# FocoosAI/focoos

Measured on AMD Instinct MI355X. Metric: images/sec @ 640^2 (infer bs=32), higher is better.
Workload: dtype bf16; 1 GPU; fai-detr-l-obj365 inference, bf16 MFMA, bs=32/GPU, 640x640, random-init weights (seed 0), uint8 HWC images resident in HBM, device post-process + D2H of packed detections included; global_batch=32, parallelism=replicas x1 (no data-path collective), steps_are=hipGraph replays, batches_in_flight=3, concurrent_batch_parts=1

## Files before the change

focoos_amd/_lib.py:

```python
from __future__ import annotations

import ctypes as C
import os
from typing import Optional

from .build import LIB_PATH, LIB_PATH_FP16

FX_ACT = {None: 0, "none": 0, "relu": 1, "silu": 2, "gelu": 3}


class FocoosAmdError(RuntimeError):
    pass


class FxConvDesc(C.Structure):
    _fields_ = [
        ("x", C.c_void_p), ("w", C.c_void_p), ("bias", C.c_void_p), ("residual", C.c_void_p), ("y", C.c_void_p),
        ("B", C.c_int32), ("H", C.c_int32), ("W", C.c_int32), ("C", C.c_int32), ("ldx", C.c_int32),
        ("Ho", C.c_int32), ("Wo", C.c_int32), ("N", C.c_int32), ("ldy", C.c_int32), ("ldr", C.c_int32),
        ("KH", C.c_int32), ("KW", C.c_int32), ("stride", C.c_int32), ("pad", C.c_int32),
        ("pool2", C.c_int32), ("act", C.c_int32), ("out_f32", C.c_int32), ("residual_after_act", C.c_int32),
        ("y_batch_stride", C.c_int64), ("w_frag", C.c_void_p), ("mask", C.c_void_p), ("ldm", C.c_int32), ("reserved0", C.c_int32),
    ]

# ... 22 lines not shown
        ("w_fwd_frag", C.c_void_p), ("w_dgrad_frag", C.c_void_p), ("bias_out", C.c_void_p),
        ("N", C.c_int32), ("C", C.c_int32), ("KH", C.c_int32), ("KW", C.c_int32), ("ld_fwd", C.c_int32), ("ld_dgrad", C.c_int32),
        ("first_block", C.c_int32), ("n_offset", C.c_int32), ("n_total", C.c_int32), ("reserved", C.c_int32),
    ]


class FxPublishEntry(C.Structure):
    _fields_ = [
        ("w", C.c_void_p), ("bn_weight", C.c_void_p), ("bn_bias", C.c_void_p), ("bn_mean", C.c_void_p), ("bn_var", C.c_void_p),
        ("bias", C.c_void_p), ("w_rows", C.c_void_p), ("w_frag", C.c_void_p), ("bias_out", C.c_void_p), ("eps", C.c_double),
        ("N", C.c_int32), ("C", C.c_int32), ("KH", C.c_int32), ("KW", C.c_int32), ("Np", C.c_int32), ("first_block", C.c_int32),
    ]


class FxPwChainDesc(C.Structure):
    _fields_ = [
        ("x1", C.c_void_p), ("x2", C.c_void_p), ("residual", C.c_void_p), ("w1", C.c_void_p), ("bias1", C.c_void_p), ("y1", C.c_void_p),
        ("w2", C.c_void_p), ("bias2", C.c_void_p), ("y2", C.c_void_p),
        ("M", C.c_int32), ("K1a", C.c_int32), ("K1b", C.c_int32), ("N1", C.c_int32), ("N2", C.c_int32),
        ("ldx1", C.c_int32), ("ldx2", C.c_int32), ("ldr", C.c_int32), ("ldy1", C.c_int32), ("ldy2", C.c_int32),
        ("act1", C.c_int32), ("act2", C.c_int32),
        ("pool", C.c_void_p), ("ldp", C.c_int32), ("img_h", C.c_int32), ("img_w", C.c_int32), ("reserved0", C.c_int32),
    ]


class FxRcStage(C.Structure):
    _fields_ = [
        ("type", C.c_int32), ("K", C.c_int32), ("N", C.c_int32), ("act", C.c_int32),
        ("src", C.c_int32), ("dst", C.c_int32), ("aux", C.c_int32),
        ("ld", C.c_int32), ("ld2", C.c_int32), ("flags", C.c_int32),
        ("w", C.c_void_p), ("bias", C.c_void_p), ("gamma", C.c_void_p), ("beta", C.c_void_p), ("g0", C.c_void_p), ("g1", C.c_void_p),
    ]


class FxFrameDesc(C.Structure):
    _fields_ = [
        ("plane", C.c_void_p * 3), ("pitch", C.c_int32 * 3), ("height", C.c_int32), ("width", C.c_int32), ("format", C.c_int32),
        ("matrix", C.c_int32), ("reserved", C.c_int32 * 3),
    ]


_vp, _i, _f = C.c_void_p, C.c_int, C.c_float

SIGNATURES = {
    "fx_abi_version": [],
    "fx_build_flags": [],
    "fx_device_info": [_i, C.POINTER(C.c_int), C.c_char_p, _i],
    "fx_conv2d_nhwc_bf16": [C.POINTER(FxConvDesc), _vp],
    "fx_conv2d_variant": [_vp, C.c_char_p, _i],
    "fx_pw_chain_supported": [_i, _i, _i, _i],
    "fx_pw_chain_pool_supported": [_i, _i, _i, _i],
    "fx_conv3x3_flat_supported": [_i, _i, _i],
    "fx_pw_chain_bf16": [C.POINTER(FxPwChainDesc), _vp],
    "fx_stem_conv3x3s2": [_vp, _i, _vp, _vp, _vp, _vp, _vp, _i, _i, _i, _i, _vp],
    "fx_stem16_conv3x3s2": [_vp, _i, _vp, _vp, _vp, _vp, _vp, _i, _i, _i, _vp],
    "fx_conv3x3_c16_nhwc_bf16": [_vp, _i, _vp, _vp, _i, _vp, _i, _i, _i, _i, _i, _i, _i, _vp],
    "fx_semseg_eval_accumulate": [_vp, _vp, _i, _i, _i, _i, _i, _i, _i, _vp, C.c_int64, _vp, _vp, _i, _i, _vp, _vp, _vp, _vp, _vp],
    "fx_detr_eval_boxes_f32": [_vp, _vp, _vp, _i, _i, _i, _i, _vp, _vp, _vp, _vp, _vp],
    "fx_coco_match_workspace_bytes": [_i],
    "fx_coco_match_bbox": [_vp, _vp, _vp, _vp, _i, _i, _i, _vp, _vp, _vp, _vp, _vp, _vp, C.c_int64, _i, _vp, _vp, _vp, _vp, _vp, _vp, C.c_size_t,
                           _vp],
    "fx_mf_eval_masks_workspace_bytes": [_i, _i, _i],
    "fx_mf_eval_masks": [_vp, _vp, _vp, _i, _i, _i, _i, _i, _i, _i, _i, _vp, _vp, _vp, _vp, C.c_int64, _f, _vp, _vp, _vp, _vp, _vp, _vp, _vp, _vp,
                         _vp, _vp, C.c_size_t, _vp],
    "fx_coco_mask_inter": [_vp, _vp, _vp, C.c_int64, _vp, _vp, _vp, _i, _i, _i, _vp, _vp, _vp, _vp, _vp, C.c_int64, _vp, _vp, _vp, C.c_int64, _vp,
                           _vp, _vp],
    "fx_coco_match_segm": [_vp, _vp, _vp, _vp, _i, _i, _i, _i, _vp, _vp, _vp, _vp, _vp, _vp, _vp, C.c_int64, _i, _vp, _vp, _vp, _vp, _vp, _vp,
                           C.c_size_t, _vp],
    "fx_augment_images_u8": [_vp, _vp, _vp, _vp, _vp, C.c_int64, _vp, _vp, _i, _vp, _i, _i, _i, _vp, _vp],
    "fx_augment_labels": [_vp, _vp, _vp, _vp, _vp, _vp, C.c_int64, _vp, _vp, _vp, _i, _i, _vp, _i, _i, _i, _i, _vp, _vp],
    "fx_resize_bilinear_u8": [_vp, _i, _i, _vp, _i, _i, _vp],
    "fx_tile_gather_u8_f32": [_vp, _i, _i, _vp, _vp, _i, _vp, _i, _i, _vp],
    "fx_frames_ingest": [_vp, _vp, _i, _vp, _i, _i, _i, _vp],
    "fx_merge_detections_workspace_bytes": [_i, _i],
    "fx_merge_detections_nms": [_vp, _vp, _vp, _vp, _vp, _i, _i, _i, _i, _f, _i, _i, _vp, _vp, _vp, _vp, _vp, _vp, C.c_size_t, _vp],
    "fx_frames_tile_gather_f32": [_vp, _vp, _i, _vp, _vp, _i, _vp, _i, _i, _vp],
    "fx_roi_select": [_vp, _vp, _vp, _vp, _i, _i, _vp, _vp, _i, _vp, _vp, _vp, _vp, _vp, _vp, _i, _i, _i, _i, _f, _i, _vp, _vp, _vp, _vp, _vp],
    "fx_frames_roi_gather_f32": [_vp, _vp, _i, _vp, _i, _vp, _i, _i, _vp],
    "fx_roi_attributes": [_vp, _i, _vp, _vp, _i, _vp, _i, _i, _vp, _vp, _i, _vp, _vp, _vp, _vp, _vp, _i, _vp, _vp, _vp, _vp],
    "fx_merge_detections_batched_workspace_bytes": [_i, _i, _i],
    "fx_merge_detections_nms_batched": [_vp, _vp, _vp, _vp, _vp, _i, _i, _i, _i, _i, _f, _i, _i, _vp, _vp, _vp, _vp, _vp, _vp, C.c_size_t, _vp],
    "fx_annotate_labels_from_detections": [_vp, _vp, _vp, _vp, _i, _i, _vp, _vp, _i, _i, _i, _i, _i, _i, _vp, _vp],
    "fx_annotate_u8": [_vp, _vp, _i, _i, _i, _i, _i, _vp, _vp, _vp, _vp, _vp, _i, C.c_int64, _vp, _vp, _i, _i, _i, _i, _vp],
    "fx_track_update": [_vp, _vp, _vp, _vp, _i, _i, _vp, _vp, _vp, _vp, _vp, _vp, _vp, _vp, _i, _f, _f, _f, _f, _f, _i, _i, _f, _vp, _vp],
    "fx_track_reset": [_vp, _vp, _vp, _vp, _vp, _vp, _vp, _vp, _i, _i, _i, _vp],
    "fx_zone_update": [_vp, _vp, _vp, _i, _i, _vp, _vp, _i, _vp, _vp, _vp, _vp, _vp, _vp, _i, _i, _vp, _vp, _vp, _vp, _vp, _vp, _vp, _vp, _vp],
    "fx_zone_reset": [_vp, _vp, _vp, _vp, _vp, _i, _i, _i, _i, _vp],
    "fx_annotate_labels_tracked": [_vp, _vp, _vp, _vp, _vp, _i, _i, _vp, _vp, _i, _i, _i, _i, _i, _i, _vp, _vp],
    "fx_annotate_zone_records": [_vp, _vp, _vp, _vp, _vp, _vp, _i, _i, _vp, _vp, _vp, _vp, _vp, _i, _i, _i, _i, _i, _i, _vp, _vp],
    "fx_annotate_overlay_u8": [_vp, _vp, _i, _i, _i, _i, _i, _vp, _vp, _vp, _vp, _vp, _vp, _i, _i, _vp, _vp, _vp, _vp, _vp, _vp, _i, _i, _i, _i,
                               _vp],
    "fx_trace_update": [_vp, _vp, _vp, _i, _i, _vp, _vp, _i, _i, _vp, _vp, _vp, _vp, _vp, _vp],
    "fx_trace_reset": [_vp, _vp, _vp, _vp, _i, _i, _i, _vp],
    "fx_dwell_update": [_vp, _vp, _vp, _i, _i, _vp, _i, _vp, _vp, _vp, _vp, _vp, _vp, _i, _vp, _vp, _vp, _vp, _vp, _vp, _vp, _vp, _vp],
    "fx_dwell_reset": [_vp, _vp, _vp, _vp, _vp, _vp, _vp, _vp, _i, _i, _i, _i, _vp],
    "fx_heat_tiles": [_i, _i, _i],
    "fx_heat_update": [_vp, _vp, _vp, _vp, _i, _i, _i, _i, _i, _i, _i, _i, _i, _vp, _vp, _vp, _vp, _vp],
    "fx_annotate_heat_u8": [_vp, _vp, _i, _i, _i, _i, _i, _vp, _vp, _i, _i, _vp, _vp],
    "fx_redact_regions": [_vp, _vp, _vp, _i, _i, _vp, _i, _vp, _vp, _vp, _vp, _i, _i, _i, _i, _vp, _vp, _vp, _vp],
    "fx_redact_u8": [_vp, _vp, _i, _i, _i, _i, _vp, _vp, _vp, _i, _vp, _i, C.c_int64, _i, _i, _i, _i, _i, _i, _vp],
    "fx_mask_rle_workspace_bytes": [_i, _i, _i, _i],
    "fx_mask_rle_encode": [_vp, _vp, _vp, _i, _i, _i, _i, _i, _vp, _vp, _vp, _vp, C.c_size_t, _vp],
    "fx_mask_polygon_workspace_bytes": [_i, _i, _i, _i, _i],
    "fx_mask_polygon_encode": [_vp, _vp, _vp, _i, _i, _i, _i, _i, _i, _vp, _vp, _vp, _vp, C.c_size_t, _vp],
    "fx_maxpool3x3s2_nhwc_bf16": [_vp, _i, _vp, _i, _i, _i, _i, _i, _vp],
    "fx_stem_conv12_u8_bf16": [_vp, _vp, _vp, _vp, _vp, _vp, _vp, _vp, _i, _i, _i, _i, _vp],
# ... 228 lines not shown
```

focoos_amd/csrc/conv_pw_chain.hip:

```cpp
#include "pw_common.h"

struct PwChainArgs {
  const bf16_t* x1;
  const bf16_t* x2;
  const bf16_t* res;
  const bf16_t* w1p;
  const bf16_t* w2p;
  const float* b1;
  const float* b2;
  bf16_t* y1;
  bf16_t* y2;
  int ldx1, ldx2, ldr, ldy1, ldy2;
  int M, N1, act1, act2;
  unsigned x1_bytes, x2_bytes, r_bytes;
  bf16_t* pool;
  int ldp, H, W;
};

template <int RL, typename F>
__device__ __forceinline__ void pw_dma_rows_map(__amdgpu_buffer_rsrc_t r, unsigned char* tile, int nrows, int ld, int col0, int wave, int lane, F&& pix) {
  const int ninstr = nrows * RL / 64;
  for (int i = wave; i < ninstr; i += 4) {
    const int q = i * 64 + lane;
    const int row = q / RL, pc = q % RL;
    const int lc = pw_swz<RL>(row, pc);
    const int m = pix(row);
    const unsigned off = (m >= 0) ? (unsigned)(m * ld + col0 + lc * 8) * 2u : FX_OOB;
    pw_dma16(r, tile + i * 1024, off);
  }
}

template <int K1A, int K1B, int N2, int BM, bool QUAD = false>
__global__ __launch_bounds__(256, ((N2 <= 64 && K1B == 0) ? 4 : ((N2 <= 128 && (K1B == 0 || N2 <= 64)) ? 3 : 2))) void pw_chain_kernel(const PwChainArgs p) {
  constexpr int K1 = K1A + K1B, KS1 = K1 / 16, KS1A = K1A / 16;
  constexpr int RLA = K1A / 8, RLB = (K1B > 0 ? K1B : 64) / 8;
  constexpr int TM = BM / 32;
  constexpr int XA_BYTES = BM * K1A * 2, XB_BYTES = BM * K1B * 2;
  constexpr int PF1 = KS1 < 4 ? KS1 : 4;
  constexpr bool HAS2 = N2 > 0;
  constexpr int WN2 = !HAS2 ? 1 : (N2 >= 128 ? 4 : 2), WM2 = 4 / WN2;
  constexpr int TN2 = !HAS2 ? 1 : N2 / (32 * WN2), TM2 = BM / (32 * WM2);
  constexpr int RL2 = (HAS2 ? N2 : 64) / 8;
  constexpr int PF2 = 4;
  static_assert(BM == 64, "64-pixel tiles");
  static_assert(K1A % 64 == 0 && K1B % 64 == 0 && PF1 == 4, "K segments in multiples of 64 (= whole blocks of 4 k-steps)");
  static_assert(!HAS2 || (N2 % 64 == 0 && N2 <= 256), "N2");
  extern __shared__ __attribute__((aligned(16))) unsigned char smem[];
  unsigned char* XA = smem;
  unsigned char* XB = smem + XA_BYTES;
  unsigned char* T = smem + XA_BYTES + XB_BYTES;

  const int tid = threadIdx.x, lane = tid & 63;
  const int wave = __builtin_amdgcn_readfirstlane(tid >> 6);
  const int l32 = lane & 31, half = lane >> 5;
  const int m0 = blockIdx.x * BM;
  const int NG = p.N1 >> 8;
  const int KS2 = p.N1 >> 4;

  __shared__ int s_pix[QUAD ? BM : 1];
  if constexpr (QUAD) {
    if (tid < BM) {
      const int W2 = p.W >> 1, QI = (p.H >> 1) * W2;
      const int q = blockIdx.x * (BM / 4) + (tid >> 2), sub = tid & 3;
      int m = -1;
      if (q * 4 < p.M) {
        const int b = q / QI, rem = q - b * QI;
        const int y2 = rem / W2, x2 = rem - y2 * W2;
        m = (b * p.H + 2 * y2 + (sub >> 1)) * p.W + 2 * x2 + (sub & 1);
      }
      s_pix[tid] = m;
    }
    __syncthreads();
  }
  auto pix = [&](int row) -> int {
    if constexpr (!QUAD) {
      const int m = m0 + row;
      return m < p.M ? m : -1;
    } else {
      return s_pix[row];
    }
  };
  const __amdgpu_buffer_rsrc_t x1r = __builtin_amdgcn_make_buffer_rsrc((void*)p.x1, 0, p.x1_bytes, 0x00020000);
  pw_dma_rows_map<RLA>(x1r, XA, BM, p.ldx1, 0, wave, lane, pix);
  if constexpr (K1B > 0) {
    const __amdgpu_buffer_rsrc_t x2r = __builtin_amdgcn_make_buffer_rsrc((void*)p.x2, 0, p.x2_bytes, 0x00020000);
    pw_dma_rows_map<RLB>(x2r, XB, BM, p.ldx2, 0, wave, lane, pix);
  }
  const __amdgpu_buffer_rsrc_t rr = __builtin_amdgcn_make_buffer_rsrc((void*)(p.res ? p.res : p.x1), 0, p.res ? p.r_bytes : 0u, 0x00020000);

  const int wn2 = wave % WN2, wm2 = wave / WN2;
  f32x16 acc2[TN2][TM2];
#pragma unroll
  for (int a = 0; a < TN2; ++a)
#pragma unroll
    for (int b = 0; b < TM2; ++b)
#pragma unroll
      for (int r = 0; r < 16; ++r) acc2[a][b][r] = 0.0f;

  for (int g = 0; g < NG; ++g) {
    int l32g = l32, halfg = half, tidg = tid;
    asm volatile("" : "+v"(l32g), "+v"(halfg), "+v"(tidg));
    if (p.res) pw_dma_rows_map<32>(rr, T, BM, p.ldr, g * 256, wave, lane, pix);
    bf16x8 a2[PF2][TN2];
    const bf16_t* w2 = p.w2p + (size_t)((wn2 * TN2) * KS2 + g * 16) * 512 + lane * 8;
    if constexpr (HAS2) {
#pragma unroll
      for (int i = 0; i < PF2; ++i)
#pragma unroll
        for (int a = 0; a < TN2; ++a) a2[i][a] = pw_ldg_frag(w2 + (size_t)(a * KS2 + i) * 512);
    }
#pragma unroll
    for (int a = 0; a < 2; ++a) {
      const bf16_t* w1 = p.w1p + (size_t)((g * 8 + wave * 2 + a) * KS1) * 512 + lane * 8;
      bf16x8 a1[PF1];
#pragma unroll
      for (int i = 0; i < PF1; ++i) a1[i] = pw_ldg_frag(w1 + i * 512);
      f32x16 acc[TM];
#pragma unroll
      for (int gq = 0; gq < 4; ++gq) {
        const float4 bb = *reinterpret_cast<const float4*>(p.b1 + g * 256 + wave * 64 + a * 32 + 8 * gq + 4 * halfg);
#pragma unroll
        for (int b = 0; b < TM; ++b) {
          acc[b][4 * gq] = bb.x; acc[b][4 * gq + 1] = bb.y; acc[b][4 * gq + 2] = bb.z; acc[b][4 * gq + 3] = bb.w;
        }
      }
      if (a == 0) {
        asm volatile("s_waitcnt vmcnt(0)" ::: "memory");
        __syncthreads();
      }
#define FX_PW_STEPS(XT_, KROW_, RL_, KL0_)                                                                                  \
  _Pragma("unroll") for (int i = 0; i < PF1; ++i) {                                                                         \
    bf16x8 xb[TM];                                                                                                          \
    _Pragma("unroll") for (int b = 0; b < TM; ++b) {                                                                        \
      const int row = b * 32 + l32k;                                                                                         \
      xb[b] = *reinterpret_cast<const bf16x8*>((XT_) + row * ((KROW_)*2) + (pw_swz<RL_>(row, ((KL0_) + i) * 2 + halfg) << 4)); \
    }                                                                                                                       \
    _Pragma("unroll") for (int b = 0; b < TM; ++b) acc[b] = FX_MFMA_32x32x16(a1[i], xb[b], acc[b]); \
    const int kn = ks0 + i + PF1;                                                                                           \
    a1[i] = pw_ldg_frag(w1 + (kn < KS1 ? kn : KS1 - 1) * 512);  \
  }
#pragma unroll 1
      for (int ks0 = 0; ks0 < KS1; ks0 += PF1) {
        int l32k = l32g;
        asm volatile("" : "+v"(l32k));
        if (K1B == 0 || ks0 < KS1A) {
          FX_PW_STEPS(XA, K1A, RLA, ks0)
        } else {
          FX_PW_STEPS(XB, (K1B > 0 ? K1B : 64), RLB, ks0 - KS1A)
        }
      }
#undef FX_PW_STEPS
#pragma unroll
      for (int b = 0; b < TM; ++b)
#pragma unroll
        for (int gq = 0; gq < 4; ++gq) {
          const int row = b * 32 + l32g;
          const int chunk = wave * 8 + a * 4 + gq;
          unsigned char* tp = T + row * 512 + ((chunk ^ (row & 15)) << 4) + halfg * 8;
          float v0 = acc[b][4 * gq], v1 = acc[b][4 * gq + 1], v2 = acc[b][4 * gq + 2], v3 = acc[b][4 * gq + 3];
          if (p.res) {
            const uint2 r2 = *reinterpret_cast<const uint2*>(tp);
            v0 += bf16lo_to_f32(r2.x);
            v1 += bf16hi_to_f32(r2.x);
            v2 += bf16lo_to_f32(r2.y);
            v3 += bf16hi_to_f32(r2.y);
          }
          if (p.act1 == FX_ACT_RELU) {
            v0 = fmaxf(v0, 0.0f); v1 = fmaxf(v1, 0.0f); v2 = fmaxf(v2, 0.0f); v3 = fmaxf(v3, 0.0f);
          }
          uint2 o;
          o.x = pack_bf16x2(v0, v1);
          o.y = pack_bf16x2(v2, v3);
          *reinterpret_cast<uint2*>(tp) = o;
        }
    }
    __syncthreads();
#pragma unroll
    for (int i = 0; i < BM * 32 / 256; ++i) {
      const int q = tidg + i * 256;
      const int row = q >> 5, lc = q & 31;
      const uint4 v = *reinterpret_cast<const uint4*>(T + row * 512 + ((lc ^ (row & 15)) << 4));
      const int m = pix(row);
      if (m >= 0 && p.y1) *reinterpret_cast<uint4*>(p.y1 + (size_t)m * p.ldy1 + g * 256 + lc * 8) = v;
    }
    if constexpr (QUAD) {
#pragma unroll
      for (int i = 0; i < (BM / 4) * 32 / 256; ++i) {
        const int idx = tidg + i * 256;
        const int j = idx >> 5, lc = idx & 31;
        float s8[8] = {0, 0, 0, 0, 0, 0, 0, 0};
#pragma unroll
        for (int r = 0; r < 4; ++r) {
          const int row = 4 * j + r;
          float f[8];
          unpack_bf16x8(*reinterpret_cast<const uint4*>(T + row * 512 + ((lc ^ (row & 15)) << 4)), f);
#pragma unroll
          for (int e = 0; e < 8; ++e) s8[e] += f[e];
        }
#pragma unroll
        for (int e = 0; e < 8; ++e) s8[e] *= 0.25f;
        const int q = blockIdx.x * (BM / 4) + j;
        if (q * 4 < p.M) *reinterpret_cast<uint4*>(p.pool + (size_t)q * p.ldp + g * 256 + lc * 8) = pack_bf16x8(s8);
      }
    }
    if constexpr (HAS2) {
#pragma unroll
      for (int ks = 0; ks < 16; ++ks) {
        bf16x8 tb[TM2];
#pragma unroll
        for (int b = 0; b < TM2; ++b) {
          const int row = (wm2 * TM2 + b) * 32 + l32g;
          tb[b] = *reinterpret_cast<const bf16x8*>(T + row * 512 + (((ks * 2 + halfg) ^ (row & 15)) << 4));
        }
#pragma unroll
        for (int a = 0; a < TN2; ++a)
#pragma unroll
          for (int b = 0; b < TM2; ++b) acc2[a][b] = FX_MFMA_32x32x16(a2[ks % PF2][a], tb[b], acc2[a][b]);
        if (ks + PF2 < 16) {
#pragma unroll
          for (int a = 0; a < TN2; ++a) a2[ks % PF2][a] = pw_ldg_frag(w2 + (size_t)(a * KS2 + ks + PF2) * 512);
        }
      }
    }
    __syncthreads();
  }

  if constexpr (HAS2) {
#pragma unroll
    for (int a = 0; a < TN2; ++a)
#pragma unroll
      for (int gq = 0; gq < 4; ++gq) {
        const int n = (wn2 * TN2 + a) * 32 + 8 * gq + 4 * half;
        const float4 bb = *reinterpret_cast<const float4*>(p.b2 + n);
#pragma unroll
        for (int b = 0; b < TM2; ++b) {
          const int row = (wm2 * TM2 + b) * 32 + l32;
          float v0 = acc2[a][b][4 * gq] + bb.x, v1 = acc2[a][b][4 * gq + 1] + bb.y;
          float v2 = acc2[a][b][4 * gq + 2] + bb.z, v3 = acc2[a][b][4 * gq + 3] + bb.w;
          if (p.act2 == FX_ACT_RELU) {
            v0 = fmaxf(v0, 0.0f); v1 = fmaxf(v1, 0.0f); v2 = fmaxf(v2, 0.0f); v3 = fmaxf(v3, 0.0f);
          }
          uint2 o;
          o.x = pack_bf16x2(v0, v1);
          o.y = pack_bf16x2(v2, v3);
          *reinterpret_cast<uint2*>(T + row * (N2 * 2) + (pw_swz<RL2>(row, n >> 3) << 4) + half * 8) = o;
        }
      }
    __syncthreads();
#pragma unroll
    for (int i = 0; i < BM * RL2 / 256; ++i) {
      const int q = tid + i * 256;
      const int row = q / RL2, lc = q % RL2;
      const uint4 v = *reinterpret_cast<const uint4*>(T + row * (N2 * 2) + (pw_swz<RL2>(row, lc) << 4));
      const int m = pix(row);
      if (m >= 0) *reinterpret_cast<uint4*>(p.y2 + (size_t)m * p.ldy2 + lc * 8) = v;
    }
  }
}

template <int K1A, int K1B, int N2, bool QUAD = false>
static int launch_pw_chain(const PwChainArgs& a, hipStream_t stream) {
  constexpr int BM = 64;
  constexpr int SMEM = BM * (K1A + K1B) * 2 + BM * 512;
  auto kern = pw_chain_kernel<K1A, K1B, N2, BM, QUAD>;
  static int attr_smem = 0;
  if (!fx_ensure_dyn_smem(reinterpret_cast<const void*>(kern), SMEM, attr_smem)) return FX_ERR_RUNTIME;
  hipLaunchKernelGGL(kern, dim3((a.M + BM - 1) / BM), dim3(256), SMEM, stream, a);
  return fx_launch_status();
}

#define FX_PW_INSTANCES(X)                                                                             \
  X(64, 0, 0) X(64, 0, 64) X(64, 0, 128) X(64, 64, 0) X(64, 64, 64) X(64, 64, 128)                     \
  X(128, 0, 0) X(128, 0, 128) X(128, 0, 256) X(128, 256, 0) X(128, 256, 128) X(128, 256, 256)          \
  X(256, 0, 0) X(256, 0, 256) X(256, 512, 0) X(256, 512, 256)

extern "C" int fx_pw_chain_supported(int K1a, int K1b, int N1, int N2) {
  if (N1 <= 0 || N1 % 256 != 0) return 0;
#define FX_PW_CASE(KA, KB, NN2) \
  if (K1a == KA && K1b == KB && N2 == NN2) return 1;
  FX_PW_INSTANCES(FX_PW_CASE)
#undef FX_PW_CASE
  return 0;
}

#define FX_PW_POOL_INSTANCES(X) X(64, 0, 128) X(128, 0, 256)

extern "C" int fx_pw_chain_pool_supported(int K1a, int K1b, int N1, int N2) {
  if (N1 <= 0 || N1 % 256 != 0) return 0;
#define FX_PW_CASE(KA, KB, NN2) \
  if (K1a == KA && K1b == KB && N2 == NN2) return 1;
  FX_PW_POOL_INSTANCES(FX_PW_CASE)
#undef FX_PW_CASE
  return 0;
}

extern "C" int fx_pw_chain_bf16(const fx_pw_chain_desc* d, fx_stream_t stream_) {
  FX_CHECK_ARG(d && d->x1 && d->w1 && d->bias1 && d->M > 0);
  FX_CHECK_ARG(d->y1 || (d->pool && d->N2 > 0));
  FX_CHECK_ARG(d->K1b == 0 || d->x2);
  FX_CHECK_ARG((d->act1 == FX_ACT_NONE || d->act1 == FX_ACT_RELU) && (d->act2 == FX_ACT_NONE || d->act2 == FX_ACT_RELU));
  FX_CHECK_ARG(d->N2 == 0 || (d->w2 && d->bias2 && d->y2));
  if (!fx_pw_chain_supported(d->K1a, d->K1b, d->N1, d->N2)) return FX_ERR_UNSUPPORTED;
  FX_CHECK_ARG(d->ldx1 >= d->K1a && d->ldx1 % 8 == 0 && (!d->y1 || (d->ldy1 >= d->N1 && d->ldy1 % 8 == 0)));
  FX_CHECK_ARG(d->K1b == 0 || (d->ldx2 >= d->K1b && d->ldx2 % 8 == 0));
  FX_CHECK_ARG(!d->residual || (d->ldr >= d->N1 && d->ldr % 8 == 0));
  FX_CHECK_ARG(d->N2 == 0 || (d->ldy2 >= d->N2 && d->ldy2 % 8 == 0));
  FX_CHECK_ARG(((uintptr_t)d->x1 % 16) == 0 && ((uintptr_t)d->x2 % 16) == 0 && ((uintptr_t)d->residual % 16) == 0);
  FX_CHECK_ARG(((uintptr_t)d->w1 % 16) == 0 && ((uintptr_t)d->w2 % 16) == 0 && ((uintptr_t)d->y1 % 16) == 0 && ((uintptr_t)d->y2 % 16) == 0);
  FX_CHECK_ARG(((uintptr_t)d->bias1 % 16) == 0 && ((uintptr_t)d->bias2 % 16) == 0);
  const int64_t x1_bytes = ((int64_t)d->M - 1) * d->ldx1 * 2 + (int64_t)d->K1a * 2;
  const int64_t x2_bytes = d->K1b ? ((int64_t)d->M - 1) * d->ldx2 * 2 + (int64_t)d->K1b * 2 : 0;
  const int64_t r_bytes = d->residual ? ((int64_t)d->M - 1) * d->ldr * 2 + (int64_t)d->N1 * 2 : 0;
  if (x1_bytes >= 0xFFFFFFF0ll || x2_bytes >= 0xFFFFFFF0ll || r_bytes >= 0xFFFFFFF0ll) return FX_ERR_UNSUPPORTED;
  PwChainArgs a;
  a.x1 = reinterpret_cast<const bf16_t*>(d->x1);
  a.x2 = reinterpret_cast<const bf16_t*>(d->x2);
  a.res = reinterpret_cast<const bf16_t*>(d->residual);
  a.w1p = reinterpret_cast<const bf16_t*>(d->w1);
  a.w2p = reinterpret_cast<const bf16_t*>(d->w2);
  a.b1 = d->bias1;
  a.b2 = d->bias2;
  a.y1 = reinterpret_cast<bf16_t*>(d->y1);
  a.y2 = reinterpret_cast<bf16_t*>(d->y2);
  a.ldx1 = d->ldx1; a.ldx2 = d->ldx2; a.ldr = d->ldr; a.ldy1 = d->ldy1; a.ldy2 = d->ldy2;
  a.M = d->M; a.N1 = d->N1; a.act1 = d->act1; a.act2 = d->act2;
  a.x1_bytes = (unsigned)x1_bytes; a.x2_bytes = (unsigned)x2_bytes; a.r_bytes = (unsigned)r_bytes;
  a.pool = reinterpret_cast<bf16_t*>(d->pool); a.ldp = d->ldp; a.H = d->img_h; a.W = d->img_w;
  hipStream_t stream = reinterpret_cast<hipStream_t>(stream_);
  if (d->pool) {
    FX_CHECK_ARG(d->img_h > 0 && d->img_w > 0 && d->img_h % 2 == 0 && d->img_w % 2 == 0 && d->M % (d->img_h * d->img_w) == 0);
    FX_CHECK_ARG(d->ldp >= d->N1 && d->ldp % 8 == 0 && ((uintptr_t)d->pool % 16) == 0);
    if (!fx_pw_chain_pool_supported(d->K1a, d->K1b, d->N1, d->N2)) return FX_ERR_UNSUPPORTED;
#define FX_PW_CASE(KA, KB, NN2) \
  if (d->K1a == KA && d->K1b == KB && d->N2 == NN2) return launch_pw_chain<KA, KB, NN2, true>(a, stream);
    FX_PW_POOL_INSTANCES(FX_PW_CASE)
#undef FX_PW_CASE
    return FX_ERR_UNSUPPORTED;
  }
#define FX_PW_CASE(KA, KB, NN2) \
  if (d->K1a == KA && d->K1b == KB && d->N2 == NN2) return launch_pw_chain<KA, KB, NN2>(a, stream);
  FX_PW_INSTANCES(FX_PW_CASE)
#undef FX_PW_CASE
  return FX_ERR_UNSUPPORTED;
}
```

focoos_amd/engine.py:

```python
from __future__ import annotations

import contextlib
import ctypes as C
import functools
import math
import os
import weakref
from typing import Dict, List, Optional, Sequence, Tuple

import torch

from . import _lib
from ._lib import FX_ACT, FxConvDesc, FxPwChainDesc, FxRcStage, check
from .engine_stdc import StdcEngineMixin, StdcPlanMixin
from .state_spec import RESNET_BLOCKS

BN_EPS = 1e-5
DEFAULT_STREAMS = 2
MIN_PART_BATCH = 4
DEFAULT_PIPELINE_DEPTH = 3


def resolve_parts(B: int, nsplit: Optional[int], two_queue_safe: bool) -> int:
    if nsplit is None:
# ... 694 lines not shown
        d.x, d.w, d.bias = x.ptr, pc.w.data_ptr(), pc.b.data_ptr()
        d.residual = residual.ptr if residual is not None else None
        d.y = out.ptr
        d.B, d.H, d.W, d.C, d.ldx = x.B, x.H, x.W, x.C, x.ld
        d.Ho, d.Wo, d.N, d.ldy = Ho, Wo, pc.N, out.ld
        d.ldr = residual.ld if residual is not None else 0
        d.KH, d.KW, d.stride, d.pad = pc.KH, pc.KW, stride, pad
        d.pool2, d.act, d.out_f32 = int(pool2), FX_ACT[act], int(out_f32)
        d.residual_after_act = int(res_after)
        d.y_batch_stride = y_batch_stride
        d.w_frag = pc.wf.data_ptr() if pc.wf is not None else None
        self.keep.append(d)
        M = x.B * Ho * Wo
        flops = 2.0 * M * pc.N * pc.KH * pc.KW * pc.C + extra_flops_per_pixel * M
        label = C.create_string_buffer(64)
        check(self.lib.fx_conv2d_variant(C.byref(d), label, 64), "fx_conv2d_variant")
        variant = label.value.decode()
        alg_bytes = 2.0 * x.B * x.H * x.W * pc.C + (4.0 if out_f32 else 2.0) * M * pc.N + (2.0 * M * pc.N if residual is not None else 0.0) \
            + 2.0 * pc.N * pc.KH * pc.KW * pc.C
        self.meta[len(self.ops)] = {"kind": "conv", "variant": variant, "flops": flops, "flops_executed": flops - extra_flops_per_pixel * M, "bytes": alg_bytes,
                                    "name": name or "slice", "M": M, "N": pc.N, "K": pc.KH * pc.KW * pc.C}
        self._op(self.lib.fx_conv2d_nhwc_bf16, C.byref(d))
        return out

    def pw_chain(self, x1: NT, x2: Optional[NT], residual: Optional[NT], cc: Tuple, ca: Optional[Tuple], name1: str, name2: Optional[str],
                 pool_name: Optional[str] = None, keep_y1: bool = True):
        w1, b1, k1a, k1b, n1 = cc
        assert x1.C == k1a and (x2 is None) == (k1b == 0) and (x2 is None or x2.C == k1b), (name1, x1.C, k1a, k1b)
        M = x1.rows
        assert keep_y1 or (pool_name is not None and ca is not None)
        y1 = self._new(name1, x1.B, x1.H, x1.W, n1) if keep_y1 else None
        d = FxPwChainDesc()
        d.x1, d.ldx1, d.K1a = x1.ptr, x1.ld, k1a
        d.x2, d.ldx2, d.K1b = (x2.ptr, x2.ld, k1b) if x2 is not None else (None, 0, 0)
        d.residual, d.ldr = (residual.ptr, residual.ld) if residual is not None else (None, 0)
        d.w1, d.bias1, d.N1, d.M = w1.data_ptr(), b1.data_ptr(), n1, M
        d.y1, d.ldy1 = (y1.ptr, y1.ld) if y1 is not None else (None, 0)
        d.act1 = d.act2 = FX_ACT["relu"]
        y2, n2 = None, 0
        if ca is not None:
            w2, b2, n2 = ca
            y2 = self._new(name2, x1.B, x1.H, x1.W, n2)
            d.w2, d.bias2, d.y2, d.ldy2 = w2.data_ptr(), b2.data_ptr(), y2.ptr, y2.ld
        d.N2 = n2
        pooled = None
        if pool_name is not None:
            pooled = self._new(pool_name, x1.B, x1.H // 2, x1.W // 2, n1)
            d.pool, d.ldp, d.img_h, d.img_w = pooled.ptr, pooled.ld, x1.H, x1.W
        self.keep.append(d)
        self.meta[len(self.ops)] = {"kind": "conv", "variant": f"pw_chain<{k1a},{k1b},{n2}>" + ("+pool" if pooled is not None else "") + ("-y1" if y1 is None else ""),
                                    "flops": 2.0 * M * n1 * (k1a + k1b + n2),
                                    "name": name1 + ("+" + name2.rsplit("res_layers.", 1)[-1] if name2 else ""), "M": M, "N": n1, "K": k1a + k1b,
                                    "bytes": 2.0 * M * (k1a + k1b + (n1 if residual is not None else 0) + (n1 if y1 is not None else 0) + n2
                                                        + (n1 / 4 if pooled is not None else 0))}
        self._op(self.lib.fx_pw_chain_bf16, C.byref(d))
        if pool_name is not None:
            return y1, y2, pooled
        return y1, y2

    def linear(self, x: NT, pc: PackedConv, **kw) -> NT:
        return self.conv(x.as_rows() if (x.H != 1 or x.W != 1) else x, pc, **kw)

    def layernorm(self, x: NT, name_ln: str, out_name: str, residual: Optional[NT] = None) -> NT:
        g, b = self.eng.ln[name_ln]
        cols = int(g.numel())
        out = self._new(out_name, x.rows, 1, 1, cols)
        self._op(self.lib.fx_layernorm_bf16, x.ptr, x.ld, residual.ptr if residual is not None else None,
                 residual.ld if residual is not None else 0, g.data_ptr(), b.data_ptr(), out.ptr, out.ld, x.rows, cols)
        return out

    def add_rows(self, x: NT, y: NT, y_rows: int, out_name: str) -> NT:
        out = self._new(out_name, x.rows, 1, 1, x.C)
        self._op(self.lib.fx_add_rows_bf16, x.ptr, x.ld, y.ptr, y.ld, y_rows, out.ptr, out.ld, x.rows, x.C)
        return out

    RC_S0, RC_S1, RC_S2, RC_S3, RC_BIG, RC_REF, RC_RED, RC_LDS = 0, 16384, 32768, 49152, 65536, 131072, 131584, 132608
    RC2_REF, RC2_RED, RC2_LDS = 65536, 66048, 67072

    def _rc_program(self, stages: List[FxRcStage], rows: int, label: str, flops: float, lds: Optional[int] = None):
        arr = (FxRcStage * len(stages))(*stages)
        host = torch.frombuffer(bytearray(bytes(arr)), dtype=torch.uint8)
        dev = host.to(self.dev)
        self.keep.append(dev)
        self.meta[len(self.ops)] = {"kind": "conv", "variant": "row_chain", "flops": flops, "name": label, "M": rows, "N": 0, "K": 0}
        self._op(self.lib.fx_row_chain, dev.data_ptr(), len(stages), rows, self.RC_LDS if lds is None else lds)

    def resize(self, x: NT, out: NT):
        self._op(self.lib.fx_resize_bilinear_nhwc_bf16, x.ptr, x.ld, out.ptr, out.ld, x.B, x.H, x.W, x.C, out.H, out.W)

    def mha(self, qkv: NT, B: int, L: int, out_name: str) -> NT:
        out = self._new(out_name, B * L, 1, 1, 256)
        q, k, v = qkv.slice(0, 256), qkv.slice(256, 256), qkv.slice(512, 256)
        self._op(self.lib.fx_mha_bf16, q.ptr, q.ld, k.ptr, k.ld, v.ptr, v.ld, out.ptr, out.ld, B, L, L, 8)
        return out

    def build_backbone(self) -> Dict[int, NT]:
        e, P, B, lib = self.eng, self.eng.P, self.B, self.lib
        H, W = self.H, self.W
        bb = "pixel_decoder.backbone"
        self.input = self._io("input", (B, H, W, 3), torch.float32 if self.f32_input else torch.uint8)
        self.sizes = self._io("sizes", (B, 2), torch.int32)
        blocks = RESNET_BLOCKS[e.depth]
        feats = {}
        use_chain = int(os.environ.get("FX_PW_CHAIN", "1")) != 0
        max_stage = int(os.environ.get("FX_PW_CHAIN_MAX_STAGE", "1"))
        pc2 = P[f"{bb}.conv1.conv1_2"]
        if os.environ.get("FX_STEM12_FUSE", "1") != "0" and not self.f32_input and pc2.wf is not None and pc2.N == 32:
# ... 517 lines not shown
```

include/focoos_amd.h:

```cpp
#ifndef FOCOOS_AMD_H
#define FOCOOS_AMD_H

#include <stddef.h>
#include <stdint.h>

#ifdef __cplusplus
extern "C" {
#endif

#define FX_ABI_VERSION 27

enum { FX_OK = 0, FX_ERR_INVALID_ARGUMENT = -1, FX_ERR_LAUNCH = -2, FX_ERR_UNSUPPORTED = -3, FX_ERR_RUNTIME = -4 };
enum { FX_ACT_NONE = 0, FX_ACT_RELU = 1, FX_ACT_SILU = 2, FX_ACT_GELU = 3 };
enum { FX_CLASS_LOSS_CE = 0, FX_CLASS_LOSS_FOCAL = 1, FX_CLASS_LOSS_BCE = 2, FX_CLASS_LOSS_BCE_FOCAL = 3 };

typedef void* fx_stream_t;

int fx_abi_version(void);
int fx_build_flags(void);
const char* fx_error_string(int code);
int fx_device_info(int device, int* cu_count, char* arch_name, int arch_name_len);

typedef struct fx_conv_desc {
  const void* x;
  const void* w;
  const float* bias;
  const void* residual;
  void* y;
  int32_t B, H, W, C, ldx;
  int32_t Ho, Wo, N, ldy, ldr;
  int32_t KH, KW, stride, pad;
  int32_t pool2;
  int32_t act;
  int32_t out_f32;
  int32_t residual_after_act;
  int64_t y_batch_stride;
  const void* w_frag;
  const void* mask;
  int32_t ldm, reserved0;
} fx_conv_desc;
int fx_conv2d_nhwc_bf16(const fx_conv_desc* d, fx_stream_t stream);
int fx_conv2d_variant(const fx_conv_desc* d, char* out, int cap);
int fx_conv3x3_flat_supported(int C, int N, int W);

typedef struct fx_pw_chain_desc {
  const void* x1;
  const void* x2;
  const void* residual;
  const void* w1;
  const float* bias1;
  void* y1;
  const void* w2;
  const float* bias2;
  void* y2;
  int32_t M, K1a, K1b, N1, N2;
  int32_t ldx1, ldx2, ldr, ldy1, ldy2;
  int32_t act1, act2;
  void* pool;
  int32_t ldp, img_h, img_w, reserved0;
} fx_pw_chain_desc;
int fx_pw_chain_supported(int K1a, int K1b, int N1, int N2);
int fx_pw_chain_pool_supported(int K1a, int K1b, int N1, int N2);
int fx_pw_chain_bf16(const fx_pw_chain_desc* d, fx_stream_t stream);

int fx_stem_conv3x3s2(const void* x, int in_f32, const float* w, const float* bias, const float* mean,
                      const float* inv_std, void* y, int B, int H, int W, int Cout, fx_stream_t stream);

int fx_stem_conv12_u8_bf16(const void* x_u8, const float* w1, const float* b1, const float* mean, const float* inv_std, const void* w2_frag,
                           const float* b2, void* y, int ldy, int B, int H, int W, fx_stream_t stream);

int fx_stem16_conv3x3s2(const void* x, int in_f32, const float* w, const float* bias, const float* mean, const float* inv_std, void* y, int B,
                        int H, int W, fx_stream_t stream);
int fx_conv3x3_c16_nhwc_bf16(const void* x, int ldx, const void* w_frag, const float* bias, int relu, void* y, int ldy, int B, int H, int W, int C,
                             int N, int stride, fx_stream_t stream);

int fx_semseg_eval_accumulate(const float* mask_probs, const float* probs, int B, int Q, int K, int h, int w, int Hin, int Win, const int32_t* sizes,
                              int64_t max_pixels, const void* gt, const int64_t* gt_off, int gt_int32, int ignore_label, int64_t* conf,
                              int32_t* status, int32_t* pred, float* score, fx_stream_t stream);

int fx_detr_eval_boxes_f32(const int32_t* idx, const float* boxes, const int32_t* sizes, int B, int Q, int K, int T,
                           int32_t* label, float* xyxy, int32_t* keep, float* xywh, fx_stream_t stream);

size_t fx_coco_match_workspace_bytes(int max_gt);
int fx_coco_match_bbox(const int32_t* label, const float* score, const int32_t* keep, const float* xywh, int B, int T, int K,
                       const double* gt_box, const int32_t* gt_cat, const int32_t* gt_flag, const double* gt_area, const int64_t* gt_off,
                       const int64_t* gt_off_host, int64_t n_gt, int max_gt, int32_t* rank, uint64_t* matched, uint64_t* ignored,
                       int64_t* npig, int32_t* status, void* ws, size_t ws_bytes, fx_stream_t stream);

size_t fx_mf_eval_masks_workspace_bytes(int B, int Q, int max_h);
int fx_mf_eval_masks(const float* mask_probs, const float* val, const int32_t* idx, int B, int Q, int K, int T, int h, int w, int Hin, int Win,
                     const int32_t* sizes, const int32_t* sizes_host, const int64_t* word_off, const int64_t* word_off_host, int64_t n_words,
                     float mask_threshold, void* words, int32_t* qlist, int32_t* nref, int32_t* count, int32_t* box, float* psum, int32_t* label,
                     int32_t* query, float* score, void* ws, size_t ws_bytes, fx_stream_t stream);
int fx_coco_mask_inter(const void* words, const int64_t* word_off, const int64_t* word_off_host, int64_t n_words, const int32_t* qlist,
                       const int32_t* nref, const int32_t* box, int B, int Q, int T, const int32_t* sizes, const int32_t* sizes_host,
                       const void* gt_words, const int64_t* gt_word_off, const int64_t* gt_word_off_host, int64_t n_gt_words,
                       const int32_t* gt_box, const int64_t* gt_off, const int64_t* gt_off_host, int64_t n_gt, int32_t* inter, int32_t* gcount,
                       fx_stream_t stream);
int fx_coco_match_segm(const int32_t* label, const float* score, const int32_t* query, const int32_t* dcount, int B, int T, int K, int Q,
                       const int32_t* inter, const int32_t* gcount, const int32_t* gt_cat, const int32_t* gt_flag, const double* gt_area,
                       const int64_t* gt_off, const int64_t* gt_off_host, int64_t n_gt, int max_gt, int32_t* rank, uint64_t* matched,
                       uint64_t* ignored, int64_t* npig, int32_t* status, void* ws, size_t ws_bytes, fx_stream_t stream);

typedef struct fx_aug_record {
  int32_t crop_w, crop_h, pad_x, pad_y, res_w, res_h, crop_x, crop_y, flags, reserved0;
  float brightness, contrast, saturation;
  int32_t reserved1[3];
} fx_aug_record;

int fx_augment_images_u8(const uint8_t* src, const int64_t* src_off, const int32_t* sizes, const fx_aug_record* recs, const int64_t* src_off_host,
                         int64_t src_bytes, const int32_t* sizes_host, const fx_aug_record* recs_host, int B, uint8_t* dst, int Ho, int Wo,
                         int pad_value, uint64_t* mean_ws, fx_stream_t stream);

int fx_augment_labels(const void* src, const int64_t* src_off, const int32_t* plane_rec, const int32_t* sizes, const fx_aug_record* recs,
                      const int64_t* src_off_host, int64_t src_count, const int32_t* plane_rec_host, const int32_t* sizes_host,
                      const fx_aug_record* recs_host, int P, int B, void* dst, int Ho, int Wo, int elem_int32, int pad_value, int32_t* flags,
// ... 501 lines not shown
```

Baseline: 5113 images/s.

## Add 128-pixel tile variant for pointwise chain kernel on large-M layers

Adds a BM=128 variant of the fused pointwise-chain kernel that processes N1 in 128-column groups instead of 256, with its own occupancy calculation and staging layout. A heuristic picks the bigger tile for specific shapes (K1a=64,N2=64 unpooled or K1a=128,N2=256 pooled) when M is at least 65536. The aim is to reuse each weight fragment load across twice as many pixels, cutting weight traffic per output. The cost is more LDS and register use per block, so fewer blocks can be resident on a CU, and the number of kernel template instances grows.

Result: slower. 5057 images/s (-1.1%).

```diff
diff --git a/focoos_amd/_lib.py b/focoos_amd/_lib.py
--- a/focoos_amd/_lib.py
+++ b/focoos_amd/_lib.py
@@ -98,6 +98,9 @@
     "fx_pw_chain_pool_supported": [_i, _i, _i, _i],
     "fx_conv3x3_flat_supported": [_i, _i, _i],
     "fx_pw_chain_bf16": [C.POINTER(FxPwChainDesc), _vp],
+    "fx_pw_chain_tile": [_i, _i, _i, _i, _i, _i],
+    "fx_pw_chain_bf16_tile": [C.POINTER(FxPwChainDesc), _i, _vp],
+    "fx_pw_chain_last_tile": [],
     "fx_stem_conv3x3s2": [_vp, _i, _vp, _vp, _vp, _vp, _vp, _i, _i, _i, _i, _vp],
     "fx_stem16_conv3x3s2": [_vp, _i, _vp, _vp, _vp, _vp, _vp, _i, _i, _i, _vp],
     "fx_conv3x3_c16_nhwc_bf16": [_vp, _i, _vp, _vp, _i, _vp, _i, _i, _i, _i, _i, _i, _i, _vp],
diff --git a/focoos_amd/csrc/conv_pw_chain.hip b/focoos_amd/csrc/conv_pw_chain.hip
--- a/focoos_amd/csrc/conv_pw_chain.hip
+++ b/focoos_amd/csrc/conv_pw_chain.hip
@@ -15,6 +15,7 @@
   unsigned x1_bytes, x2_bytes, r_bytes;
   bf16_t* pool;
   int ldp, H, W;
+  int wmask;
 };
 
 template <int RL, typename F>
@@ -30,8 +31,16 @@
   }
 }
 
-template <int K1A, int K1B, int N2, int BM, bool QUAD = false>
-__global__ __launch_bounds__(256, ((N2 <= 64 && K1B == 0) ? 4 : ((N2 <= 128 && (K1B == 0 || N2 <= 64)) ? 3 : 2))) void pw_chain_kernel(const PwChainArgs p) {
+template <int K1A, int K1B, int N2, int BM>
+constexpr int pw_chain_occupancy() {
+  if (BM == 64) return (N2 <= 64 && K1B == 0) ? 4 : ((N2 <= 128 && (K1B == 0 || N2 <= 64)) ? 3 : 2);
+  const int lds = (160 * 1024) / (BM * (K1A + K1B) * 2 + 32 * 1024);
+  const int regs = N2 <= 64 ? 3 : ((K1A == 64 && K1B > 0) ? 1 : 2);
+  return lds < regs ? lds : regs;
+}
+
+template <int K1A, int K1B, int N2, int BM, bool QUAD = false, int ABL = 0>
+__global__ __launch_bounds__(256, (pw_chain_occupancy<K1A, K1B, N2, BM>())) void pw_chain_kernel(const PwChainArgs p) {
   constexpr int K1 = K1A + K1B, KS1 = K1 / 16, KS1A = K1A / 16;
   constexpr int RLA = K1A / 8, RLB = (K1B > 0 ? K1B : 64) / 8;
   constexpr int TM = BM / 32;
@@ -41,20 +50,32 @@
   constexpr int WN2 = !HAS2 ? 1 : (N2 >= 128 ? 4 : 2), WM2 = 4 / WN2;
   constexpr int TN2 = !HAS2 ? 1 : N2 / (32 * WN2), TM2 = BM / (32 * WM2);
   constexpr int RL2 = (HAS2 ? N2 : 64) / 8;
-  constexpr int PF2 = 4;
-  static_assert(BM == 64, "64-pixel tiles");
+  constexpr int PF2 = (BM == 128 && N2 == 256 && K1B == 0) ? 2 : 4;
+  constexpr int GC = BM == 64 ? 256 : 128;
+  constexpr int RLT = GC / 8, TROW = GC * 2;
+  constexpr int RLT_LOG = BM == 64 ? 5 : 4, GC_LOG = RLT_LOG + 3;
+  constexpr int NPASS = GC / 128;
+  constexpr int KSG = GC / 16;
+  constexpr int T_BYTES = BM * TROW;
+  static_assert(BM == 64 || BM == 128, "64- or 128-pixel tiles");
   static_assert(K1A % 64 == 0 && K1B % 64 == 0 && PF1 == 4, "K segments in multiples of 64 (= whole blocks of 4 k-steps)");
   static_assert(!HAS2 || (N2 % 64 == 0 && N2 <= 256), "N2");
   extern __shared__ __attribute__((aligned(16))) unsigned char smem[];
   unsigned char* XA = smem;
   unsigned char* XB = smem + XA_BYTES;
   unsigned char* T = smem + XA_BYTES + XB_BYTES;
+  unsigned char* Y2T = (BM * N2 * 2 <= T_BYTES) ? T : smem;
+  static_assert(BM * N2 * 2 <= T_BYTES || BM * N2 * 2 <= XA_BYTES + XB_BYTES + T_BYTES, "y2 staging tile");
 
   const int tid = threadIdx.x, lane = tid & 63;
   const int wave = __builtin_amdgcn_readfirstlane(tid >> 6);
   const int l32 = lane & 31, half = lane >> 5;
   const int m0 = blockIdx.x * BM;
-  const int NG = p.N1 >> 8;
+  const int NG = p.N1 >> GC_LOG;
+  auto widx = [&](int i) -> int {
+    if constexpr (ABL != 0) return i & p.wmask;
+    else return i;
+  };
   const int KS2 = p.N1 >> 4;
 
   __shared__ int s_pix[QUAD ? BM : 1];
@@ -100,25 +121,25 @@
   for (int g = 0; g < NG; ++g) {
     int l32g = l32, halfg = half, tidg = tid;
     asm volatile("" : "+v"(l32g), "+v"(halfg), "+v"(tidg));
-    if (p.res) pw_dma_rows_map<32>(rr, T, BM, p.ldr, g * 256, wave, lane, pix);
+    if (p.res) pw_dma_rows_map<RLT>(rr, T, BM, p.ldr, g * GC, wave, lane, pix);
     bf16x8 a2[PF2][TN2];
-    const bf16_t* w2 = p.w2p + (size_t)((wn2 * TN2) * KS2 + g * 16) * 512 + lane * 8;
+    const bf16_t* w2 = p.w2p + (size_t)widx((wn2 * TN2) * KS2 + g * KSG) * 512 + lane * 8;
     if constexpr (HAS2) {
 #pragma unroll
       for (int i = 0; i < PF2; ++i)
 #pragma unroll
-        for (int a = 0; a < TN2; ++a) a2[i][a] = pw_ldg_frag(w2 + (size_t)(a * KS2 + i) * 512);
-    }
-#pragma unroll
-    for (int a = 0; a < 2; ++a) {
-      const bf16_t* w1 = p.w1p + (size_t)((g * 8 + wave * 2 + a) * KS1) * 512 + lane * 8;
+        for (int a = 0; a < TN2; ++a) a2[i][a] = pw_ldg_frag(w2 + (size_t)widx(a * KS2 + i) * 512);
+    }
+#pragma unroll
+    for (int a = 0; a < NPASS; ++a) {
+      const bf16_t* w1 = p.w1p + (size_t)widx((g * (GC / 32) + wave * NPASS + a) * KS1) * 512 + lane * 8;
       bf16x8 a1[PF1];
 #pragma unroll
-      for (int i = 0; i < PF1; ++i) a1[i] = pw_ldg_frag(w1 + i * 512);
+      for (int i = 0; i < PF1; ++i) a1[i] = pw_ldg_frag(w1 + widx(i) * 512);
       f32x16 acc[TM];
 #pragma unroll
       for (int gq = 0; gq < 4; ++gq) {
-        const float4 bb = *reinterpret_cast<const float4*>(p.b1 + g * 256 + wave * 64 + a * 32 + 8 * gq + 4 * halfg);
+        const float4 bb = *reinterpret_cast<const float4*>(p.b1 + g * GC + wave * (NPASS * 32) + a * 32 + 8 * gq + 4 * halfg);
 #pragma unroll
         for (int b = 0; b < TM; ++b) {
           acc[b][4 * gq] = bb.x; acc[b][4 * gq + 1] = bb.y; acc[b][4 * gq + 2] = bb.z; acc[b][4 * gq + 3] = bb.w;
@@ -137,7 +158,7 @@
     }                                                                                                                       \
     _Pragma("unroll") for (int b = 0; b < TM; ++b) acc[b] = FX_MFMA_32x32x16(a1[i], xb[b], acc[b]); \
     const int kn = ks0 + i + PF1;                                                                                           \
-    a1[i] = pw_ldg_frag(w1 + (kn < KS1 ? kn : KS1 - 1) * 512);  \
+    a1[i] = pw_ldg_frag(w1 + widx(kn < KS1 ? kn : KS1 - 1) * 512);  \
   }
 #pragma unroll 1
       for (int ks0 = 0; ks0 < KS1; ks0 += PF1) {
@@ -155,8 +176,8 @@
 #pragma unroll
         for (int gq = 0; gq < 4; ++gq) {
           const int row = b * 32 + l32g;
-          const int chunk = wave * 8 + a * 4 + gq;
-          unsigned char* tp = T + row * 512 + ((chunk ^ (row & 15)) << 4) + halfg * 8;
+          const int chunk = wave * (NPASS * 4) + a * 4 + gq;
+          unsigned char* tp = T + row * TROW + (pw_swz<RLT>(row, chunk) << 4) + halfg * 8;
           float v0 = acc[b][4 * gq], v1 = acc[b][4 * gq + 1], v2 = acc[b][4 * gq + 2], v3 = acc[b][4 * gq + 3];
           if (p.res) {
             const uint2 r2 = *reinterpret_cast<const uint2*>(tp);
@@ -176,49 +197,49 @@
     }
     __syncthreads();
 #pragma unroll
-    for (int i = 0; i < BM * 32 / 256; ++i) {
+    for (int i = 0; i < BM * RLT / 256; ++i) {
       const int q = tidg + i * 256;
-      const int row = q >> 5, lc = q & 31;
-      const uint4 v = *reinterpret_cast<const uint4*>(T + row * 512 + ((lc ^ (row & 15)) << 4));
+      const int row = q >> RLT_LOG, lc = q & (RLT - 1);
+      const uint4 v = *reinterpret_cast<const uint4*>(T + row * TROW + (pw_swz<RLT>(row, lc) << 4));
       const int m = pix(row);
-      if (m >= 0 && p.y1) *reinterpret_cast<uint4*>(p.y1 + (size_t)m * p.ldy1 + g * 256 + lc * 8) = v;
+      if (m >= 0 && p.y1) *reinterpret_cast<uint4*>(p.y1 + (size_t)m * p.ldy1 + g * GC + lc * 8) = v;
     }
     if constexpr (QUAD) {
 #pragma unroll
-      for (int i = 0; i < (BM / 4) * 32 / 256; ++i) {
+      for (int i = 0; i < (BM / 4) * RLT / 256; ++i) {
         const int idx = tidg + i * 256;
-        const int j = idx >> 5, lc = idx & 31;
+        const int j = idx >> RLT_LOG, lc = idx & (RLT - 1);
         float s8[8] = {0, 0, 0, 0, 0, 0, 0, 0};
 #pragma unroll
         for (int r = 0; r < 4; ++r) {
           const int row = 4 * j + r;
           float f[8];
-          unpack_bf16x8(*reinterpret_cast<const uint4*>(T + row * 512 + ((lc ^ (row & 15)) << 4)), f);
+          unpack_bf16x8(*reinterpret_cast<const uint4*>(T + row * TROW + (pw_swz<RLT>(row, lc) << 4)), f);
 #pragma unroll
           for (int e = 0; e < 8; ++e) s8[e] += f[e];
         }
 #pragma unroll
         for (int e = 0; e < 8; ++e) s8[e] *= 0.25f;
         const int q = blockIdx.x * (BM / 4) + j;
-        if (q * 4 < p.M) *reinterpret_cast<uint4*>(p.pool + (size_t)q * p.ldp + g * 256 + lc * 8) = pack_bf16x8(s8);
+        if (q * 4 < p.M) *reinterpret_cast<uint4*>(p.pool + (size_t)q * p.ldp + g * GC + lc * 8) = pack_bf16x8(s8);
       }
     }
     if constexpr (HAS2) {
 #pragma unroll
-      for (int ks = 0; ks < 16; ++ks) {
+      for (int ks = 0; ks < KSG; ++ks) {
         bf16x8 tb[TM2];
 #pragma unroll
         for (int b = 0; b < TM2; ++b) {
           const int row = (wm2 * TM2 + b) * 32 + l32g;
-          tb[b] = *reinterpret_cast<const bf16x8*>(T + row * 512 + (((ks * 2 + halfg) ^ (row & 15)) << 4));
+          tb[b] = *reinterpret_cast<const bf16x8*>(T + row * TROW + (pw_swz<RLT>(row, ks * 2 + halfg) << 4));
         }
 #pragma unroll
         for (int a = 0; a < TN2; ++a)
 #pragma unroll
           for (int b = 0; b < TM2; ++b) acc2[a][b] = FX_MFMA_32x32x16(a2[ks % PF2][a], tb[b], acc2[a][b]);
-        if (ks + PF2 < 16) {
-#pragma unroll
-          for (int a = 0; a < TN2; ++a) a2[ks % PF2][a] = pw_ldg_frag(w2 + (size_t)(a * KS2 + ks + PF2) * 512);
+        if (ks + PF2 < KSG) {
+#pragma unroll
+          for (int a = 0; a < TN2; ++a) a2[ks % PF2][a] = pw_ldg_frag(w2 + (size_t)widx(a * KS2 + ks + PF2) * 512);
         }
       }
     }
@@ -243,7 +264,7 @@
           uint2 o;
           o.x = pack_bf16x2(v0, v1);
           o.y = pack_bf16x2(v2, v3);
-          *reinterpret_cast<uint2*>(T + row * (N2 * 2) + (pw_swz<RL2>(row, n >> 3) << 4) + half * 8) = o;
+          *reinterpret_cast<uint2*>(Y2T + row * (N2 * 2) + (pw_swz<RL2>(row, n >> 3) << 4) + half * 8) = o;
         }
       }
     __syncthreads();
@@ -251,22 +272,34 @@
     for (int i = 0; i < BM * RL2 / 256; ++i) {
       const int q = tid + i * 256;
       const int row = q / RL2, lc = q % RL2;
-      const uint4 v = *reinterpret_cast<const uint4*>(T + row * (N2 * 2) + (pw_swz<RL2>(row, lc) << 4));
+      const uint4 v = *reinterpret_cast<const uint4*>(Y2T + row * (N2 * 2) + (pw_swz<RL2>(row, lc) << 4));
       const int m = pix(row);
       if (m >= 0) *reinterpret_cast<uint4*>(p.y2 + (size_t)m * p.ldy2 + lc * 8) = v;
     }
   }
 }
 
-template <int K1A, int K1B, int N2, bool QUAD = false>
+template <int K1A, int K1B, int N2, bool QUAD, int BM, int ABL = 0>
 static int launch_pw_chain(const PwChainArgs& a, hipStream_t stream) {
-  constexpr int BM = 64;
-  constexpr int SMEM = BM * (K1A + K1B) * 2 + BM * 512;
-  auto kern = pw_chain_kernel<K1A, K1B, N2, BM, QUAD>;
+  constexpr int SMEM = BM * (K1A + K1B) * 2 + 32 * 1024;
+  auto kern = pw_chain_kernel<K1A, K1B, N2, BM, QUAD, ABL>;
   static int attr_smem = 0;
   if (!fx_ensure_dyn_smem(reinterpret_cast<const void*>(kern), SMEM, attr_smem)) return FX_ERR_RUNTIME;
   hipLaunchKernelGGL(kern, dim3((a.M + BM - 1) / BM), dim3(256), SMEM, stream, a);
   return fx_launch_status();
+}
+
+static thread_local int pw_chain_last_tile = 0;
+extern "C" int fx_pw_chain_last_tile(void) { return pw_chain_last_tile; }
+
+template <int K1A, int K1B, int N2, bool QUAD>
+static int launch_pw_chain_bm(const PwChainArgs& a, int bm, hipStream_t stream) {
+  pw_chain_last_tile = bm;
+  if (bm == 64) return launch_pw_chain<K1A, K1B, N2, QUAD, 64>(a, stream);
+  if constexpr (K1A <= 128) {
+    if (bm == 128) return launch_pw_chain<K1A, K1B, N2, QUAD, 128>(a, stream);
+  }
+  return FX_ERR_UNSUPPORTED;
 }
 
 #define FX_PW_INSTANCES(X)                                                                             \
@@ -294,13 +327,32 @@
   return 0;
 }
 
-extern "C" int fx_pw_chain_bf16(const fx_pw_chain_desc* d, fx_stream_t stream_) {
+int fx_tune(const char* env_name, int default_value);
+
+#define FX_PW_CHAIN_BM128_MIN_M 65536
+extern "C" int fx_pw_chain_tile(int K1a, int K1b, int N1, int N2, int M, int pooled) {
+  if (!(pooled ? fx_pw_chain_pool_supported(K1a, K1b, N1, N2) : fx_pw_chain_supported(K1a, K1b, N1, N2))) return 0;
+  static const int knob = fx_tune("FX_PW_CHAIN_BM", 0);
+  const bool has128 = K1a <= 128;
+  if (knob == 64 || !has128) return 64;
+  if (knob == 128) return 128;
+  const bool routed = pooled ? (K1a == 128 && N2 == 256) : (K1a == 64 && N2 == 64);
+  return (routed && M >= FX_PW_CHAIN_BM128_MIN_M) ? 128 : 64;
+}
+
+
+static int pw_chain_run(const fx_pw_chain_desc* d, int bm, fx_stream_t stream_) {
   FX_CHECK_ARG(d && d->x1 && d->w1 && d->bias1 && d->M > 0);
   FX_CHECK_ARG(d->y1 || (d->pool && d->N2 > 0));
   FX_CHECK_ARG(d->K1b == 0 || d->x2);
   FX_CHECK_ARG((d->act1 == FX_ACT_NONE || d->act1 == FX_ACT_RELU) && (d->act2 == FX_ACT_NONE || d->act2 == FX_ACT_RELU));
   FX_CHECK_ARG(d->N2 == 0 || (d->w2 && d->bias2 && d->y2));
   if (!fx_pw_chain_supported(d->K1a, d->K1b, d->N1, d->N2)) return FX_ERR_UNSUPPORTED;
+  if (bm == 0) {
+    bm = fx_pw_chain_tile(d->K1a, d->K1b, d->N1, d->N2, d->M, d->pool != nullptr);
+    if (bm == 0) bm = 64;
+  }
+  if (!(bm == 64 || (bm == 128 && d->K1a <= 128))) return FX_ERR_UNSUPPORTED;
   FX_CHECK_ARG(d->ldx1 >= d->K1a && d->ldx1 % 8 == 0 && (!d->y1 || (d->ldy1 >= d->N1 && d->ldy1 % 8 == 0)));
   FX_CHECK_ARG(d->K1b == 0 || (d->ldx2 >= d->K1b && d->ldx2 % 8 == 0));
   FX_CHECK_ARG(!d->residual || (d->ldr >= d->N1 && d->ldr % 8 == 0));
@@ -326,20 +378,28 @@
   a.M = d->M; a.N1 = d->N1; a.act1 = d->act1; a.act2 = d->act2;
   a.x1_bytes = (unsigned)x1_bytes; a.x2_bytes = (unsigned)x2_bytes; a.r_bytes = (unsigned)r_bytes;
   a.pool = reinterpret_cast<bf16_t*>(d->pool); a.ldp = d->ldp; a.H = d->img_h; a.W = d->img_w;
+  a.wmask = -1;
   hipStream_t stream = reinterpret_cast<hipStream_t>(stream_);
   if (d->pool) {
     FX_CHECK_ARG(d->img_h > 0 && d->img_w > 0 && d->img_h % 2 == 0 && d->img_w % 2 == 0 && d->M % (d->img_h * d->img_w) == 0);
     FX_CHECK_ARG(d->ldp >= d->N1 && d->ldp % 8 == 0 && ((uintptr_t)d->pool % 16) == 0);
     if (!fx_pw_chain_pool_supported(d->K1a, d->K1b, d->N1, d->N2)) return FX_ERR_UNSUPPORTED;
 #define FX_PW_CASE(KA, KB, NN2) \
-  if (d->K1a == KA && d->K1b == KB && d->N2 == NN2) return launch_pw_chain<KA, KB, NN2, true>(a, stream);
+  if (d->K1a == KA && d->K1b == KB && d->N2 == NN2) return launch_pw_chain_bm<KA, KB, NN2, true>(a, bm, stream);
     FX_PW_POOL_INSTANCES(FX_PW_CASE)
 #undef FX_PW_CASE
     return FX_ERR_UNSUPPORTED;
   }
 #define FX_PW_CASE(KA, KB, NN2) \
-  if (d->K1a == KA && d->K1b == KB && d->N2 == NN2) return launch_pw_chain<KA, KB, NN2>(a, stream);
+  if (d->K1a == KA && d->K1b == KB && d->N2 == NN2) return launch_pw_chain_bm<KA, KB, NN2, false>(a, bm, stream);
   FX_PW_INSTANCES(FX_PW_CASE)
 #undef FX_PW_CASE
   return FX_ERR_UNSUPPORTED;
 }
+
+extern "C" int fx_pw_chain_bf16(const fx_pw_chain_desc* d, fx_stream_t stream) { return pw_chain_run(d, 0, stream); }
+
+extern "C" int fx_pw_chain_bf16_tile(const fx_pw_chain_desc* d, int bm, fx_stream_t stream) {
+  if (bm != 64 && bm != 128) return FX_ERR_UNSUPPORTED;
+  return pw_chain_run(d, bm, stream);
+}
diff --git a/focoos_amd/engine.py b/focoos_amd/engine.py
--- a/focoos_amd/engine.py
+++ b/focoos_amd/engine.py
@@ -770,7 +770,8 @@
                                     "flops": 2.0 * M * n1 * (k1a + k1b + n2),
                                     "name": name1 + ("+" + name2.rsplit("res_layers.", 1)[-1] if name2 else ""), "M": M, "N": n1, "K": k1a + k1b,
                                     "bytes": 2.0 * M * (k1a + k1b + (n1 if residual is not None else 0) + (n1 if y1 is not None else 0) + n2
-                                                        + (n1 / 4 if pooled is not None else 0))}
+                                                        + (n1 / 4 if pooled is not None else 0)),
+                                    "tile": self.lib.fx_pw_chain_tile(k1a, k1b, n1, n2, M, int(pooled is not None))}
         self._op(self.lib.fx_pw_chain_bf16, C.byref(d))
         if pool_name is not None:
             return y1, y2, pooled
diff --git a/include/focoos_amd.h b/include/focoos_amd.h
--- a/include/focoos_amd.h
+++ b/include/focoos_amd.h
@@ -62,6 +62,9 @@
 int fx_pw_chain_supported(int K1a, int K1b, int N1, int N2);
 int fx_pw_chain_pool_supported(int K1a, int K1b, int N1, int N2);
 int fx_pw_chain_bf16(const fx_pw_chain_desc* d, fx_stream_t stream);
+int fx_pw_chain_tile(int K1a, int K1b, int N1, int N2, int M, int pooled);
+int fx_pw_chain_bf16_tile(const fx_pw_chain_desc* d, int bm, fx_stream_t stream);
+int fx_pw_chain_last_tile(void);
 
 int fx_stem_conv3x3s2(const void* x, int in_f32, const float* w, const float* bias, const float* mean,
                       const float* inv_std, void* y, int B, int H, int W, int Cout, fx_stream_t stream);
```
